# data-mermaid/mermaid-classifier

Measured on AMD Instinct MI355X. Metric: patches/sec (224x224 EfficientNet-B0), higher is better.
Workload: dtype f16; 1 GPU; EfficientNet-B0 forward, batch=256 random 224x224 u8 patches per GPU -> (256,1280) fp32; per_gpu_batch=256, global_batch=256, weights=synthetic seed 0, input_batches_rotated=8, lanes_per_gpu=2, parallelism=patch-sharded x1

## Files before the change

### mermaid_classifier_amd/csrc/device_common.h

```cpp
#pragma once
#include <hip/hip_runtime.h>
#include <stdint.h>
#include <stdlib.h>
#include <algorithm>
#include <atomic>
#include <type_traits>

#include "kernels.h"

typedef _Float16 h8 __attribute__((ext_vector_type(8)));
typedef _Float16 h4 __attribute__((ext_vector_type(4)));
typedef float f4 __attribute__((ext_vector_type(4)));
typedef float f2 __attribute__((ext_vector_type(2)));

static __device__ __forceinline__ float sigmoid_f(float x) { return __builtin_amdgcn_rcpf(1.0f + __expf(-x)); }
static __device__ __forceinline__ float silu_f(float x) { return x * sigmoid_f(x); }
static __device__ __forceinline__ float silu_scaled(float t)
{
    return t * __builtin_amdgcn_rcpf(1.0f + __builtin_amdgcn_exp2f(-t));
}

static __device__ __forceinline__ uint32_t cvt_pk_f16(float a, float b)
{
    uint32_t d;
// ... 87 lines not shown
typedef uint32_t u4v __attribute__((ext_vector_type(4)));
template <typename T>
static __device__ __forceinline__ const GLOBAL_AS T* sgpr_ptr(const void* p)
{
    const uint64_t v = reinterpret_cast<uint64_t>(p);
    const uint32_t lo = __builtin_amdgcn_readfirstlane((uint32_t)v), hi = __builtin_amdgcn_readfirstlane((uint32_t)(v >> 32));
    return reinterpret_cast<const GLOBAL_AS T*>(((uint64_t)hi << 32) | lo);
}
template <typename T>
static __device__ __forceinline__ T gload(const GLOBAL_AS void* base, unsigned byte_off)
{
    return *reinterpret_cast<const GLOBAL_AS T*>(reinterpret_cast<const GLOBAL_AS char*>(base) + byte_off);
}
#define T7_BAR() asm volatile("s_waitcnt lgkmcnt(0)\n\ts_barrier" ::: "memory")

#define LAUNCH_CHECK()                          \
    do {                                        \
        hipError_t e__ = hipGetLastError();     \
        if (e__ != hipSuccess) return (int)e__; \
    } while (0)

template <auto Kernel>
static int set_max_lds(int bytes)
{
    static std::atomic<bool> done[64];
    int dev = 0;
    if (hipGetDevice(&dev) != hipSuccess) dev = 0;
    const bool tracked = dev >= 0 && dev < 64;
    if (tracked && done[dev].load(std::memory_order_acquire)) return 0;
    const hipError_t e = hipFuncSetAttribute(reinterpret_cast<const void*>(Kernel), hipFuncAttributeMaxDynamicSharedMemorySize, bytes);
// ... 32 lines not shown
```

### mermaid_classifier_amd/csrc/k_early.hip

```cpp
#include "device_common.h"

template <int KSTEPS, bool RES>
__global__ __launch_bounds__(256) void thin_proj_kernel(const _Float16* __restrict__ X, int K, const _Float16* __restrict__ Wp,
                                                        const float* __restrict__ bias, _Float16* __restrict__ Y, int N,
                                                        const float* __restrict__ gate, int HW, int frags_per_wg,
                                                        const _Float16* __restrict__ res, int plane_rows)
{
    const int tid = threadIdx.x, lane = tid & 63, wave = tid >> 6;
    const int m = lane & 15, q = lane >> 4;
    const int b = blockIdx.y;
    const int nfrag = HW >> 4;
    const int f0 = blockIdx.x * frags_per_wg;
    const int f1 = f0 + frags_per_wg < nfrag ? f0 + frags_per_wg : nfrag;
    const int cbase = q * 8;
    const int cres = cbase < N ? cbase : 0;
    const _Float16* xb = X + (size_t)b * HW * K;
    auto load = [&](int f, h8 (&dst)[KSTEPS], h8& r) {
        const size_t row = (size_t)f * 16 + m;
#pragma unroll
        for (int ks = 0; ks < KSTEPS; ++ks) {
            const int k0 = ks * 32 + q * 8, k = k0 < K ? k0 : K - 8;
            dst[ks] = plane_rows ? *reinterpret_cast<const h8*>(X + (((size_t)(k >> 5) * plane_rows + (size_t)b * HW + row) * 32 + (k & 31)))
                                 : *reinterpret_cast<const h8*>(xb + row * K + k);
        }
        if (RES) r = *reinterpret_cast<const h8*>(res + ((size_t)b * HW + row) * N + cres);
    };
    h8 xc[KSTEPS], xn[KSTEPS], rc = {0, 0, 0, 0, 0, 0, 0, 0}, rn = rc;
    int f = f0 + wave;
    load(f < f1 ? f : f1 - 1, xc, rc);
    h8 wf[KSTEPS][2];
    {
        f4 g0[KSTEPS], g1[KSTEPS];
        uint4 wr[KSTEPS][2];
#pragma unroll
        for (int ks = 0; ks < KSTEPS; ++ks) {
            const int k0 = ks * 32 + q * 8, k = k0 < K ? k0 : K - 8;
            g0[ks] = *reinterpret_cast<const f4*>(gate + (size_t)b * K + k);
            g1[ks] = *reinterpret_cast<const f4*>(gate + (size_t)b * K + k + 4);
        }
#pragma unroll
        for (int ks = 0; ks < KSTEPS; ++ks)
#pragma unroll
            for (int t = 0; t < 2; ++t) wr[ks][t] = *reinterpret_cast<const uint4*>(Wp + ((size_t)(ks * 2 + t) * 64 + lane) * 8);
#pragma unroll
        for (int ks = 0; ks < KSTEPS; ++ks)
#pragma unroll
// ... 17 lines not shown
#pragma unroll
            for (int j = 0; j < 4; ++j) {
                o[j] = (_Float16)(a0[j] + (RES ? (float)rc[j] : 0.f));
                o[4 + j] = (_Float16)(a1[j] + (RES ? (float)rc[4 + j] : 0.f));
            }
            *reinterpret_cast<h8*>(Y + ((size_t)b * HW + (size_t)f * 16 + m) * N + cbase) = o;
        }
        if (more) {
#pragma unroll
            for (int ks = 0; ks < KSTEPS; ++ks) xc[ks] = xn[ks];
            rc = rn;
        }
    }
}

template <bool PLANAR>
__global__ __launch_bounds__(512, 4) void mb1_kernel(Mb1Args a)
{
    constexpr int WC = 58, NPOS = 17 * WC, NPF = (NPOS + 15) / 16, ES2 = 160;
    extern __shared__ __attribute__((aligned(16))) unsigned char smem[];
    unsigned char* E = smem;
    float* pred = reinterpret_cast<float*>(smem + NPF * 8 * ES2);
    const int tid = threadIdx.x, lane = tid & 63, wave = __builtin_amdgcn_readfirstlane(tid >> 6);
    const int m = lane & 15, q = lane >> 4;
    const int tile = blockIdx.x, b = blockIdx.z;
    const int ty = tile >> 1, tx = tile & 1;
    const int oy0 = 8 * ty, ox0 = 28 * tx, iy0 = 16 * ty, ix0 = 56 * tx;
    const GLOBAL_AS _Float16* xg = sgpr_ptr<_Float16>(a.X) + (size_t)b * 112 * 112 * 32;
    uint2 xbp[8];
    {
        u4v xr[8];
#pragma unroll
        for (int i = 0; i < 8; ++i) {
            const int pf = wave + 8 * i;
            const int p = 16 * pf + m;
            const int r = p / WC, c = p - r * WC;
            const int iy = iy0 + r, ix = ix0 + c;
            const bool ok = pf < NPF && p < NPOS && iy < 112 && ix < 112;
            xr[i] = gload<u4v>(xg, (unsigned)((((ok ? iy : 0) * 112 + (ok ? ix : 0)) * 32 + 8 * q) * 2));
        }
        const uint4 wraw = *reinterpret_cast<const uint4*>(a.pre_w + lane * 8);
        const f4 bpre = *reinterpret_cast<const f4*>(a.pre_b + 4 * q);
        const f4 g0 = *reinterpret_cast<const f4*>(a.pre_gate + (size_t)b * 32 + 8 * q);
        const f4 g1 = *reinterpret_cast<const f4*>(a.pre_gate + (size_t)b * 32 + 8 * q + 4);
        const uint4 wgated = gate_h8(wraw, g0, g1);
        const h8 wpre = *reinterpret_cast<const h8*>(&wgated);
#pragma unroll
        for (int i = 0; i < 8; ++i) {
            const f4 x1 = __builtin_amdgcn_mfma_f32_16x16x32_f16(wpre, *reinterpret_cast<const h8*>(&xr[i]), bpre, 0, 0, 0);
            h4 xh;
#pragma unroll
            for (int j = 0; j < 4; ++j) xh[j] = (_Float16)x1[j];
            xbp[i] = *reinterpret_cast<const uint2*>(&xh);
        }
    }
    h4 wexp[2];
    float bexp[2];
    float kdw[9], dbias;
    auto request_chunk = [&](int chunk) {
// ... 828 lines not shown
    __syncthreads();
    if (tid < 32) {
        float sum = 0.f;
#pragma unroll
        for (int s0 = 0; s0 < 64; s0 += 16) {
            float pv[16];
#pragma unroll
            for (int ss = 0; ss < 16; ++ss) pv[ss] = red[(s0 + ss) * 32 + tid];
#pragma unroll
            for (int ss = 0; ss < 16; ++ss) sum += pv[ss];
        }
        pool_part[((size_t)b * 49 + ty * 7 + tx) * 32 + tid] = sum;
    }
}

template <int KSTEPS, bool RES>
static int launch_thin_proj_t(const GemmArgs& a, hipStream_t st)
{
    const int nfrag = a.HW / 16, patches = a.M / a.HW;
    int per = (int)(((long)nfrag * patches / 2048 + 3) / 4 * 4);
    if (per < 8) per = 8;
    if (per > 112) per = 112;
    if (nfrag < per) per = nfrag;
    dim3 grid((nfrag + per - 1) / per, patches);
    hipLaunchKernelGGL((thin_proj_kernel<KSTEPS, RES>), grid, dim3(256), 0, st, a.X, a.K, a.Wp, a.bias, a.Y, a.N, a.gate, a.HW, per, a.res,
                       a.x_plane_rows);
    LAUNCH_CHECK();
    return 0;
}

#define TP(KSTEPS, RES) {{KSTEPS, RES}, "thin_proj", launch_thin_proj_t<KSTEPS, RES != 0>},
static const Inst<2, GemmArgs> THIN_PROJ_TABLE[] = {TP(1, 1) TP(2, 0) TP(3, 0) TP(5, 0) TP(5, 1)};
#undef TP

const char* thin_proj_label(int ksteps, int res) { return inst_label(THIN_PROJ_TABLE, {ksteps, res}); }

int launch_thin_proj(const GemmArgs& a, int patches, hipStream_t st)
{
    if (a.nt != 2 || a.n_chunks != 1 || a.K > 192 || (a.K & 7) || a.N > 32 || (a.N & 7) || (a.HW & 15) || !a.gate || a.epi != EPI_LINEAR ||
        a.M != patches * a.HW || (a.x_plane_rows && (a.x_plane_rows != a.M || (a.K & 31))))
        return -15;
    return inst_launch(THIN_PROJ_TABLE, {a.Kp / 32, a.res ? 1 : 0}, a, st, -15);
}

int launch_stem_dw(const uint8_t* patches, const _Float16* w, const float* bias, const float* padval, const float* Wdw,
                   const float* bdw, _Float16* out, float* pool_part, int B, hipStream_t st)
{
    hipLaunchKernelGGL(stem_dw_kernel, dim3(7, 7, B), dim3(256), 0, st, patches, w, bias, padval, Wdw, bdw, out, pool_part);
    LAUNCH_CHECK();
    return 0;
}

int launch_mb1(const Mb1Args& a, hipStream_t st)
{
    if (a.B < 1) return -15;
    const int lds = 62 * 8 * 160 + 16 * 32 * 4;
    if (int r = set_max_lds<&mb1_kernel<false>>(lds)) return r;
    if (int r = set_max_lds<&mb1_kernel<true>>(lds)) return r;
    if (a.planar) hipLaunchKernelGGL(mb1_kernel<true>, dim3(14, 1, a.B), dim3(512), lds, st, a);
    else hipLaunchKernelGGL(mb1_kernel<false>, dim3(14, 1, a.B), dim3(512), lds, st, a);
    LAUNCH_CHECK();
    return 0;
}

template <int KSD, int CKS, int CE, int HIMG>
static int launch_mbt_t(const MbtArgs& a, hipStream_t st)
{
    constexpr int NROWS = 14 + 2 * (KSD / 2), WW = HIMG == 28 ? 28 : 30, NPF = (NROWS * WW + 15) / 16;
    const int lds = NPF * 16 * 112 + 10 * 48 * 4;
    if (int r = set_max_lds<&mbt_kernel<KSD, CKS, CE, HIMG>>(lds)) return r;
    hipLaunchKernelGGL((mbt_kernel<KSD, CKS, CE, HIMG>), dim3((HIMG / 14) * (HIMG / 28), CE / 48, a.B), dim3(512), lds, st, a);
    LAUNCH_CHECK();
    return 0;
}

template <int CKS, int CE>
static int launch_mbt4_t(const MbtArgs& a, hipStream_t st)
// ... 46 lines not shown
```

### mermaid_classifier_amd/csrc/k_generic.hip

```cpp
#include "device_common.h"

#define STEM_TILE 16
#define STEM_IN (2 * STEM_TILE + 1)
#define STEM_ROWH 104

template <int NT>
__global__ __launch_bounds__(256) void stem_conv_kernel(const uint8_t* __restrict__ patches,
                                                        const _Float16* __restrict__ w,
                                                        const float* __restrict__ bias,
                                                        const float* __restrict__ padval,
                                                        _Float16* __restrict__ out)
{
    __shared__ __attribute__((aligned(16))) _Float16 tile[STEM_IN * STEM_ROWH];
    const int tx = blockIdx.x, ty = blockIdx.y, b = blockIdx.z;
    const int tid = threadIdx.x;
    const uint8_t* img = patches + (size_t)b * (224 * 224 * 3);
    const int iy0 = ty * 32, ix0 = tx * 32;
    const float pv0 = padval[0], pv1 = padval[1], pv2 = padval[2];
    for (int i = tid; i < STEM_IN * 25; i += 256) {
        const int r = i / 25, d = i - r * 25;
        const int iy = iy0 + r;
        const int boff = ix0 * 3 + d * 4;
        uint32_t word = 0;
        const bool row_ok = iy < 224;
// ... 561 lines not shown
                *reinterpret_cast<f4*>(gate + (size_t)row * C + n) = o;
            }
        }
    }
}

__global__ __launch_bounds__(256) void se_small_kernel(const float* __restrict__ pool_part, int nparts, int C, int Cs,
                                                       const float* __restrict__ wr,
                                                       const float* __restrict__ br,
                                                       const float* __restrict__ we,
                                                       const float* __restrict__ be,
                                                       float* __restrict__ gate)
{
    __shared__ float pooled[256];
    __shared__ float rs[16];
    const int tid = threadIdx.x, lane = tid & 63, wave = tid >> 6;
    const int b = blockIdx.x;
    if (tid < C) {
        const float* pp = pool_part + (size_t)b * nparts * C + tid;
        float s0 = 0.f, s1 = 0.f, s2 = 0.f, s3 = 0.f;
        int p = 0;
#pragma unroll 4
        for (; p + 3 < nparts; p += 4) {
            s0 += pp[(size_t)p * C];
            s1 += pp[(size_t)(p + 1) * C];
            s2 += pp[(size_t)(p + 2) * C];
            s3 += pp[(size_t)(p + 3) * C];
        }
        for (; p < nparts; ++p) s0 += pp[(size_t)p * C];
        pooled[tid] = (s0 + s1) + (s2 + s3);
    }
    __syncthreads();
    for (int j = wave; j < Cs; j += 4) {
        float s = 0.f;
        for (int c = lane; c < C; c += 64) s = __builtin_fmaf(pooled[c], wr[(size_t)j * C + c], s);
#pragma unroll
        for (int o = 32; o >= 1; o >>= 1) s += __shfl_xor(s, o);
        if (lane == 0) rs[j] = silu_f(s + br[j]);
    }
    __syncthreads();
    if (tid < C) {
        float acc = be[tid];
        for (int j = 0; j < Cs; ++j) acc = __builtin_fmaf(rs[j], we[(size_t)tid * Cs + j], acc);
        gate[(size_t)b * C + tid] = sigmoid_f(acc);
    }
}

__global__ __launch_bounds__(1024) void se_wide_kernel(const float* __restrict__ pool_part, int nparts, int C, int Cs,
                                                      const float* __restrict__ wr,
                                                      const float* __restrict__ br,
                                                      const float* __restrict__ we,
                                                      const float* __restrict__ be,
                                                      float* __restrict__ gate)
{
    extern __shared__ float se_sm[];
    float* pooled = se_sm;
    float* rs = se_sm + C;
    const int tid = threadIdx.x, lane = tid & 63, wave = tid >> 6;
    const int b = blockIdx.x;
    for (int c = tid; c < C; c += 1024) {
// ... 573 lines not shown
```

### mermaid_classifier_amd/csrc/kernels.h

```cpp
#pragma once
#include <hip/hip_runtime.h>
#include <stdint.h>

enum { EPI_SILU = 0, EPI_LINEAR = 1, EPI_GAP = 2 };


int mmc_fail(int code, const char* fmt, ...);

struct GemmArgs {
    const _Float16* X;
    int M, K;
    const _Float16* Wp;
    int Kp;
    const float* bias;
    _Float16* Y;
    int N;
    int mt, nt, n_chunks, defer_gate;
    int epi;
    const float* gate;
    int HW;
    const _Float16* res;
    float* gap_out;
    int x_plane_rows;
    float inv_hw;
};

struct Fp8GemmArgs {
    const _Float16* X;
    int M, K;
    const uint8_t* W8;
    int KS128, NFp;
    const float* sw;
    const float* bias;
    _Float16* Y;
    int N;
    const float* gate;
    int HW;
    const _Float16* res;
// ... 64 lines not shown
    const _Float16* pre_wproj;
    const float* pre_bproj;
    const _Float16* head_w;
    const float* head_b;
    float* feat;
    float inv_hw;
    int in_wide;
};
int launch_tail7(const TailArgs& a, hipStream_t st);

struct Mb1Args {
    const _Float16* X;
    const _Float16* pre_w;
    const float* pre_b;
    const float* pre_gate;
    const _Float16* wexp;
    const float* bexp;
    const float* wdw;
    const float* bdw;
    _Float16* D;
    int planar;
    float* pool;
    int B;
};
int launch_mb1(const Mb1Args& a, hipStream_t st);

struct MbtArgs {
    const _Float16* X;
    const _Float16* wexp;
    const float* bexp;
// ... 46 lines not shown
const char* proj_patch_label(int K, int N, int HW, int res);

int launch_mbconv_a(const MbArgs& a, hipStream_t st);
const char* mbconv_a_label(const MbArgs& a);
const char* mbconv_pre_label(const MbArgs& a);
const char* mbconv_d_label(const MbArgs& a);
int launch_mbconv_pre(const MbArgs& a, const _Float16* pre_w, const float* pre_b, const float* pre_gate, hipStream_t st);
int launch_mbconv_d(const MbArgs& a, hipStream_t st);
int launch_stem(const uint8_t* patches, const _Float16* w, const float* bias, const float* padval, _Float16* out, int B,
                int channels, hipStream_t st);
int launch_stem_dw(const uint8_t* patches, const _Float16* w, const float* bias, const float* padval, const float* Wdw,
                   const float* bdw, _Float16* out, float* pool_part, int B, hipStream_t st);
int launch_pw_gemm(const GemmArgs& a, hipStream_t st);
const char* pw_gemm_label(int mt, int nt, int epi, int gate, int res, int defer_gate);
int launch_thin_proj(const GemmArgs& a, int patches, hipStream_t st);
const char* thin_proj_label(int ksteps, int res);
int launch_dwconv(const DwArgs& a, hipStream_t st);
const char* dwconv_label(int ks, int stride, int tw);
int launch_se_gate(const float* pool_part, int nparts, int B, int C, int Cs4, const float* WrP, const float* br,
                   const float* WeP, const float* be, float* gate, hipStream_t st);
int launch_se_small(const float* pool_part, int nparts, int B, int C, int Cs, const float* wr, const float* br,
                    const float* we, const float* be, float* gate, hipStream_t st);
int launch_se_wide(const float* pool_part, int nparts, int B, int C, int Cs, const float* wr, const float* br,
                   const float* we_t , const float* be, float* gate, hipStream_t st);
int launch_mlp_layer(const float* X, int M, int K, const float* W, const float* bias, float* Y, int N, bool relu,
                     hipStream_t st);
int launch_calibrate(const float* logits, int M, int K, const float* a, const float* b, float* proba, int32_t* argmax,
                     hipStream_t st);
int launch_calibrate_topk(const float* logits, int M, int K, const float* a, const float* b, int k, int32_t* idx, float* scores,
                          float* proba, float* rowbuf, hipStream_t st);
constexpr int EVAL_TOTALS = 5;
// ... 5 lines not shown
```

### mermaid_classifier_amd/csrc/mmc_api.cpp

```cpp
#include <hip/hip_runtime.h>

#include <algorithm>
#include <cmath>
#include <cstdarg>
#include <cstdio>
#include <cstdlib>
#include <cstring>
#include <map>
#include <mutex>
#include <thread>
#include <string>
#include <vector>

#include "../../include/mmc.h"
#include "kernels.h"
#include "trainer_internal.h"

static thread_local char g_err[512] = "";
static int fail(int code, const char* fmt, ...)
{
    va_list ap;
    va_start(ap, fmt);
    vsnprintf(g_err, sizeof g_err, fmt, ap);
    va_end(ap);
// ... 123 lines not shown
    if (small_m) {
        int best = 4, waste = 1 << 30;
        for (int nt = 4; nt >= 2; --nt) {
            const int w = (tiles + nt - 1) / nt * nt - tiles;
            if (w < waste) { waste = w; best = nt; }
        }
        return tiles <= 4 ? tiles : best;
    }
    for (int nt = 8; nt >= 1; --nt)
        if (tiles % nt == 0) return nt;
    return 1;
}

struct Options {
    bool keep, graph, tail_clk, profile_serial;
    bool fuse, fuse_b0, mb1, mbt, mbt2, mbt4, mb_dot2, mid14, mid14m, projse, se_small, thin_proj, b1_planar;
    bool tail, tail_full, tail_b11;
    int lanes, fp8_maxh;
};
static bool env_starts(const char* name, char c)
{
    const char* e = getenv(name);
    return e && e[0] == c;
}
static Options read_options()
{
    auto on = [](const char* name) { return !env_starts(name, '0'); };
    Options o;
    o.keep = env_starts("MMC_KEEP_ACTIVATIONS", '1');
    o.graph = on("MMC_GRAPH") && !o.keep;
    o.tail_clk = env_starts("MMC_TAIL_CLK", '1') && !o.keep;
    o.profile_serial = env_starts("MMC_PROFILE_SERIAL", '1');
    o.fuse = on("MMC_FUSE");
    o.fuse_b0 = on("MMC_FUSE_B0");
    o.mb1 = on("MMC_MB1");
    o.mbt = on("MMC_MBT");
    o.mbt2 = on("MMC_MBT2");
    o.mbt4 = on("MMC_MBT4");
    o.mb_dot2 = on("MMC_MB_DOT2");
    o.projse = on("MMC_PROJSE");
    o.se_small = on("MMC_SE_SMALL");
    o.thin_proj = on("MMC_THIN_PROJ");
    o.b1_planar = on("MMC_B1_PLANAR");
    o.tail = on("MMC_TAIL");
    o.tail_full = on("MMC_TAIL_FULL");
    o.tail_b11 = on("MMC_TAIL_B11");
    const char* e = getenv("MMC_MID14");
    o.mid14 = !e || atoi(e) != 0;
    e = getenv("MMC_MID14M");
    o.mid14m = !e || atoi(e) >= 1;
    e = getenv("MMC_LANES");
    o.lanes = e ? atoi(e) : 2;
    e = getenv("MMC_FP8_MAXH");
    o.fp8_maxh = e && atoi(e) > 7 ? atoi(e) : 7;
    return o;
}
// ... 24 lines not shown
    B11All,
};

struct BlockW {
    BlockDef d;
    int H = 0, Ho = 0, ce = 0, cs = 0, cs4 = 0, pad = 0;
    bool has_expand = false, skip = false;
    int tw = 0, CG = 0, S = 0, iters = 0, parts = 0, nz = 1;
    bool fusable = false;
    bool d_fits = false;
    int d_npair = 0, d_wl_off = 0, d_red_off = 0, d_lds = 0;
    MbArgs mb{};
    Front front = Front::Unfused;
    Back back = Back::SeProject;
    Se se = Se::Fused;
    Proj proj = Proj::Gemm;
    bool mbt4 = false, mid14m = false;
    bool planar = false;
    int nparts = 0;
    const char *front_label = nullptr, *back_label = nullptr;
    PwLayer expand, project;
    Fp8Layer p8;
    float *dw_w = nullptr, *dw_b = nullptr;
    float *se_br = nullptr, *se_be = nullptr;
    float *se_wrp = nullptr, *se_wep = nullptr;
    float *se_wr_nat = nullptr, *se_we_nat = nullptr, *se_br_nat = nullptr;
    _Float16* exp_nat = nullptr;
    _Float16* exp_frag = nullptr;
    uint32_t* t_dwp = nullptr;
    uint32_t* t_dwp4 = nullptr;
// ... 92 lines not shown
};

#define MMC_GRAPH_CACHE 32

struct mmc_backbone {
    int device = 0, max_batch = 0;
    int arch = MMC_ARCH_B0, nblk = 16, stem_ch = 32, head_in = 320, feat = 1280;
    Options opt;
    _Float16* stem_w = nullptr;
    float *stem_b = nullptr, *stem_pad = nullptr;
    std::vector<BlockW> blk;
    PwLayer head;
    struct Lane {
        _Float16 *act0 = nullptr, *act1 = nullptr, *expbuf = nullptr, *dwbuf = nullptr;
        float *pool_part = nullptr, *gate = nullptr;
        hipStream_t stream = nullptr;
        hipEvent_t done = nullptr;
    };
    Lane lanes[4];
    struct GraphEntry { const void* in; float* out; int n; hipGraphExec_t exec; };
    std::vector<GraphEntry> graphs;
    bool use_graph = false;
    int graph_warm = 0;
    struct SeenKey { const void* in; float* out; int n; };
    std::vector<SeenKey> seen;
    std::vector<SeenKey> evicted;
    int evictions = 0;
    long long captures = 0;
    hipStream_t gstream = nullptr;
    int nlanes = 1, lane_cap = 0;
// ... 201 lines not shown
        break;
    }
    if (family && !B.front_label)
        return fail(MMC_ERR_ARG, "block %d: no %s instantiation for %dx%d, kernel %d, stride %d, %d -> %d channels (tile %dx%d, chunk %d)",
                    i, family, B.H, B.H, B.d.k, B.d.s, B.d.cin, B.ce, B.mb.TH, B.mb.TWo, B.mb.CC);
    const bool fp8_blk = bb->fp8 && B.Ho <= o.fp8_maxh;
    const char* pp = proj_patch_label(B.ce, B.d.cout, HWo, B.skip ? 1 : 0);
    const bool proj_patch = o.fuse && o.projse && B.fusable && B.has_expand && B.cs4 <= 28 && pp && (is_b0 ? i >= 3 && i <= 10 : !fp8_blk);
    if (tail_blk || (i == 11 && bb->tail == TailRoute::B11)) B.back = Back::Tail;
    else if (proj_patch) B.back = Back::ProjPatch;
    else if (i == 0 && bb->fuse_b0b1) B.back = Back::SeFolded;
    else B.back = Back::SeProject;
    B.back_label = B.back == Back::ProjPatch ? pp : nullptr;
    B.se = !is_b0 ? Se::Wide : (o.se_small && B.ce <= 256 && B.cs <= 16) ? Se::Small : Se::Fused;
    PwLayer& P = B.project;
    const bool thin = o.thin_proj && P.nt == 2 && P.n_chunks == 1 && thin_proj_label(P.Kp / 32, B.skip ? 1 : 0) && P.N <= 32 &&
                      (P.N & 7) == 0 && (HWo & 15) == 0 && HWo >= 3136;
    B.proj = thin ? Proj::Thin : fp8_blk ? Proj::Fp8 : Proj::Gemm;
    if (B.back == Back::SeProject && B.proj == Proj::Gemm && !plan_gemm(P, EPI_LINEAR, true, B.skip, HWo))
        return fail(MMC_ERR_ARG, "block %d: no pw_gemm (project) instantiation for %d -> %d channels at %dx%d", i, B.ce, B.d.cout, B.Ho, B.Ho);
    B.planar = B.front == Front::Mb1 && thin && o.b1_planar && !o.keep && P.K == 96;
    return 0;
}

extern "C" int mmc_backbone_create_ex(const void* packed, size_t nbytes, int arch, int device, int max_batch, unsigned flags,
                                      mmc_backbone** out)
{
    if (!out) return fail(MMC_ERR_ARG, "out is NULL");
    if (flags & ~(unsigned)MMC_PRECISION_FP8) return fail(MMC_ERR_ARG, "unknown flags 0x%x", flags);
    if ((flags & MMC_PRECISION_FP8) && arch != MMC_ARCH_B4)
        return fail(MMC_ERR_ARG, "MMC_PRECISION_FP8 is implemented for MMC_ARCH_B4 (BASELINE configs[4]): B0's late blocks run fused kernels without a separate project GEMM");
    *out = nullptr;
    if (!packed || nbytes < 16) return fail(MMC_ERR_WEIGHTS, "weights blob is empty");
    if (arch != MMC_ARCH_B0 && arch != MMC_ARCH_B4) return fail(MMC_ERR_ARG, "unsupported arch %d (MMC_ARCH_B0 or MMC_ARCH_B4)", arch);
    if (max_batch < 1 || max_batch > 4096) return fail(MMC_ERR_ARG, "max_batch %d out of range [1,4096]", max_batch);
    const uint8_t* base = static_cast<const uint8_t*>(packed);
    uint32_t hdr[4];
// ... 51 lines not shown
        const std::vector<BlockW>& K = bb->blk;
        bb->fuse_stem = is_b0 && o.fuse;
        const MbArgs& m1 = K[1].mb;
        bb->fuse_b0b1 = o.fuse_b0 && bb->fuse_stem && K[0].ce == 32 && K[0].d.cout == 16 && K[1].d.cin == 16 && K[1].fusable &&
                        !(o.mb_dot2 && B0_DOT2[1] && K[1].d_fits) && m1.TH == 8 && m1.TWo == 8 && m1.CC == 48 && m1.tw == 2 &&
                        m1.pb == 1 && m1.npair == 3;
        bool t12 = is_b0 && o.fuse && o.tail && NBLK == 16;
        for (int i = 12; i <= 15 && t12; ++i)
            t12 = K[i].fusable && K[i].H == 7 && K[i].d.s == 1 && K[i].d.cin == 192 && K[i].ce == 1152 && K[i].cs == 48;
        const BlockW& B11 = K[11 < NBLK ? 11 : 0];
        const bool t11 = t12 && o.tail_full && HEAD_IN % 32 == 0 && B11.fusable && B11.ce == 672 && B11.d.cout == 192 &&
                         B11.cs4 == 28 && B11.mb.tiles_x * B11.mb.tiles_y == 1;
        const bool t11all = t11 && o.tail_b11 && !o.keep && B11.mb.ksteps == 4 && B11.d.k == 5 && B11.d.s == 2 && B11.H == 14;
        bb->tail = t11all ? TailRoute::B11All : t11 ? TailRoute::B11 : t12 ? TailRoute::B12 : TailRoute::None;
        for (int i = 0; i < NBLK; ++i) TRY_OR_FREE(plan_block(bb, bb->blk[i], i));
        bb->head.nt = 4;
        const int HWh = K[NBLK - 1].Ho * K[NBLK - 1].Ho;
        if (bb->tail != TailRoute::B11 && bb->tail != TailRoute::B11All && !plan_gemm(bb->head, EPI_GAP, false, false, HWh)) {
            mmc_backbone_destroy(bb);
            return fail(MMC_ERR_ARG, "head: no pw_gemm (average pool) instantiation for nt %d at %d pixels per patch", bb->head.nt, HWh);
        }
    }

    std::vector<uint64_t> table(2 * (size_t)nt);
    memcpy(table.data(), base + 16, (size_t)nt * 16);
    BlobReader rd{base, nbytes, nt, table.data()};
    int err = 0;
#define TAKE(var, n, what)                         \
    const float* var = rd.take((n), what, &err);   \
    if (!var) { mmc_backbone_destroy(bb); return err; }
// ... 260 lines not shown
    }
    const size_t mb = (size_t)max_batch;
    {
        int nl = std::max(1, std::min(o.lanes, 4));
        if (bb->keep || max_batch < 2 * nl) nl = 1;
        bb->nlanes = nl;
        bb->lane_cap = (max_batch + nl - 1) / nl;
        const size_t lc = (size_t)bb->lane_cap;
        for (int l = 0; l < nl; ++l) {
            mmc_backbone::Lane& L = bb->lanes[l];
            TRY_OR_FREE(dev_alloc(bb, &L.act0, lc * max_act));
            TRY_OR_FREE(dev_alloc(bb, &L.act1, lc * max_act));
            TRY_OR_FREE(dev_alloc(bb, &L.expbuf, lc * (max_exp ? max_exp : 64)));
            TRY_OR_FREE(dev_alloc(bb, &L.dwbuf, lc * max_dw));
            TRY_OR_FREE(dev_alloc(bb, &L.pool_part, lc * max_pool));
            TRY_OR_FREE(dev_alloc(bb, &L.gate, lc * (size_t)max_c));
            if (nl > 1) {
                if (hipStreamCreateWithFlags(&L.stream, hipStreamNonBlocking) != hipSuccess ||
                    hipEventCreateWithFlags(&L.done, hipEventDisableTiming) != hipSuccess) {
                    mmc_backbone_destroy(bb);
                    return fail(MMC_ERR_HIP, "cannot create internal stream/event");
                }
            }
        }
        if (nl > 1 && hipEventCreateWithFlags(&bb->fork, hipEventDisableTiming) != hipSuccess) {
            mmc_backbone_destroy(bb);
            return fail(MMC_ERR_HIP, "cannot create fork event");
        }
    }
    TRY_OR_FREE(dev_alloc(bb, &bb->in_stage, mb * (size_t)IMG * IMG * 3));
// ... 69 lines not shown
    _Float16* y = ws.act1;
    auto swap_xy = [&] { _Float16* t = x; x = y; y = t; };
    const int lane_idx = (int)(&ws - bb->lanes);
    if (!bb->fuse_stem) {
        STEP("stem", "stem_conv", launch_stem(patches_dev, bb->stem_w, bb->stem_b, bb->stem_pad, x, n, bb->stem_ch, st));
        SAVE("stem", x, (size_t)n * 112 * 112 * bb->stem_ch, true);
    }
    for (int i = 0; i < bb->nblk; ++i) {
        BlockW& B = bb->blk[i];
        if (B.front == Front::Tail) break;
        const int HWi = B.H * B.H, HWo = B.Ho * B.Ho;
        snprintf(nm, sizeof nm, "b%d.mbconv", i);
        switch (B.front) {
        case Front::StemDw:
            STEP("stem+b0.dw", "stem_dw", launch_stem_dw(patches_dev, bb->stem_w, bb->stem_b, bb->stem_pad, B.dw_w, B.dw_b,
                                                          bb->fuse_b0b1 ? y : ws.dwbuf, ws.pool_part, n, st));
            break;
        case Front::Mbt: {
            MbtArgs ta{};
            ta.X = x; ta.wexp = B.exp_frag; ta.bexp = B.expand.b; ta.dwp = B.t_dwp; ta.bdw = B.dw_b; ta.D = ws.dwbuf;
            ta.pool = ws.pool_part; ta.B = n; ta.H = B.H; ta.Cin = B.d.cin; ta.Ce = B.ce; ta.ks = B.d.k; ta.stride = B.d.s;
            ta.dwtoe = B.mbt4 ? B.dw_diag : nullptr;
            STEP(nm, B.front_label, launch_mbt(ta, st));
            break;
        }
        case Front::Mid14: {
            Mid14Args ma{};
            ma.X = x; ma.wexp = B.exp_frag; ma.bexp = B.expand.b; ma.dwp = B.t_dwp4; ma.bdw = B.dw_b; ma.D = ws.dwbuf;
            ma.pool = ws.pool_part; ma.B = n; ma.Cin = B.d.cin; ma.Ce = B.ce; ma.ks = B.d.k;
            ma.dwdiag = B.mid14m ? B.dw_diag : nullptr;
            ma.nsplit = B.mid14m ? 1 : 4;
            if (bb->mid_clk && i == 10) ma.dbg_clk = bb->mid_clk + (size_t)lane_idx * bb->lane_cap * 128;
            STEP(nm, B.front_label, launch_mid14(ma, st));
            break;
        }
        case Front::Mb1: {
            Mb1Args m1{};
            m1.X = y; m1.pre_w = bb->b0_pre_w; m1.pre_b = bb->blk[0].project.b; m1.pre_gate = ws.gate; m1.wexp = bb->b1_exp_pre;
            m1.bexp = B.expand.b; m1.wdw = B.dw_w; m1.bdw = B.dw_b; m1.D = ws.dwbuf; m1.pool = ws.pool_part; m1.B = n;
            m1.planar = B.planar ? 1 : 0;
            STEP("b0.project+b1.mbconv", "mb1", launch_mb1(m1, st));
            break;
        }
        case Front::MbPre: case Front::MbD: case Front::MbA: {
            MbArgs a = B.mb;
            a.X = x; a.Wexp = B.exp_nat; a.bexp = B.expand.b; a.Wdw = B.dw_w; a.bdw = B.dw_b; a.out = ws.dwbuf;
            a.pool_part = ws.pool_part; a.B = n;
            if (B.front == Front::MbD) {
                STEP(nm, B.front_label, launch_mbconv_d(a, st));
            } else if (B.front == Front::MbPre) {
                a.X = y; a.Cin = 32; a.Wexp = bb->b1_exp_pre;
                STEP("b0.project+b1.mbconv", B.front_label, launch_mbconv_pre(a, bb->b0_pre_w, bb->blk[0].project.b, ws.gate, st));
            } else {
                STEP(nm, B.front_label, launch_mbconv_a(a, st));
            }
            break;
// ... 26 lines not shown
            pa.dbg_clk = bb->keep ? bb->dbg_clk : nullptr;
            pa.B = n; pa.HW = HWo; pa.K = B.ce; pa.N = B.d.cout; pa.CSP = B.cs4; pa.nparts = B.nparts;
            pa.psc = (float)(1.0 / ((double)HWo * LOG2E));
            snprintf(nm, sizeof nm, "b%d.projse", i);
            STEP(nm, B.back_label, launch_proj_patch(pa, st));
            snprintf(nm, sizeof nm, "b%d.gate", i);
            SAVE(nm, ws.gate, (size_t)n * B.ce, false);
            snprintf(nm, sizeof nm, "b%d.out", i);
            SAVE(nm, y, (size_t)n * HWo * B.d.cout, true);
            snprintf(nm, sizeof nm, "b%d.clk", i);
            SAVE(nm, bb->dbg_clk, (size_t)n * 8, false);
            swap_xy();
            continue;
        }
        snprintf(nm, sizeof nm, "b%d.gate", i);
        if (B.se == Se::Wide)
            STEP(nm, "se_wide", launch_se_wide(ws.pool_part, B.nparts, n, B.ce, B.cs, B.se_wr_nat, B.se_br_nat, B.se_we_nat, B.se_be,
                                               ws.gate, st));
        else if (B.se == Se::Small)
            STEP(nm, "se_small", launch_se_small(ws.pool_part, B.nparts, n, B.ce, B.cs, B.se_wr_nat, B.se_br_nat, B.se_we_nat, B.se_be,
                                                 ws.gate, st));
        else
            STEP(nm, "se_fused", launch_se_gate(ws.pool_part, B.nparts, n, B.ce, B.cs4, B.se_wrp, B.se_br, B.se_wep, B.se_be,
                                                ws.gate, st));
        SAVE(nm, ws.gate, (size_t)n * B.ce, false);
        if (B.back == Back::SeFolded) continue;
        snprintf(nm, sizeof nm, "b%d.project", i);
        if (B.proj == Proj::Thin) {
            GemmArgs a{};
            a.X = ws.dwbuf; a.M = n * HWo; a.K = B.project.K; a.Wp = B.project.w; a.Kp = B.project.Kp; a.bias = B.project.b; a.Y = y;
            a.N = B.project.N; a.nt = B.project.nt; a.n_chunks = B.project.n_chunks; a.epi = EPI_LINEAR; a.gate = ws.gate; a.HW = HWo;
            a.res = B.skip ? x : nullptr;
            a.x_plane_rows = B.planar ? n * HWo : 0;
            STEP(nm, "thin_proj", launch_thin_proj(a, n, st));
        } else if (B.proj == Proj::Fp8) {
            Fp8GemmArgs fa{};
            fa.X = ws.dwbuf; fa.M = n * HWo; fa.K = B.p8.K; fa.W8 = B.p8.w8; fa.KS128 = B.p8.KS128; fa.NFp = B.p8.NFp; fa.sw = B.p8.sw;
            fa.bias = B.p8.b; fa.Y = y; fa.N = B.p8.N; fa.gate = ws.gate; fa.HW = HWo; fa.res = B.skip ? x : nullptr;
            STEP(nm, "pw_gemm_fp8", launch_pw_gemm_fp8(fa, st));
        } else
            STEP(nm, B.project.label[gemm_mt(B.project, n * HWo) - 1],
                 run_gemm(B.project, ws.dwbuf, n * HWo, y, EPI_LINEAR, ws.gate, HWo, B.skip ? x : nullptr, nullptr, st));
        snprintf(nm, sizeof nm, "b%d.out", i);
        SAVE(nm, y, (size_t)n * HWo * B.d.cout, true);
        swap_xy();
    }
    const float inv_hw7 = (float)(1.0 / (49.0 * LOG2E));
    if (bb->tail == TailRoute::B11All || (bb->tail == TailRoute::B11 && !bb->keep)) {
        const BlockW& B11 = bb->blk[11];
// ... 755 lines not shown
```

Baseline: 229,000 patches/s.

## Inline small squeeze-excite gate into thin projection and mb1 kernels

Adds an option that computes the small SE gate (pool reduce, reduce FC, SiLU, expand FC, sigmoid) inside each consuming workgroup of the thin projection kernel (blocks 1 and 2) and the fused b0-project+b1 kernel. This removes the separate se_small launches and the gate round-trip through global memory. In exchange, every workgroup redundantly recomputes the per-patch gate and adds LDS barriers before its main loop. The path is gated behind the MMC_SE_INLINE environment flag, and the standalone se_small kernel is refactored to share the same chain code.

```diff
diff --git a/mermaid_classifier_amd/csrc/device_common.h b/mermaid_classifier_amd/csrc/device_common.h
--- a/mermaid_classifier_amd/csrc/device_common.h
+++ b/mermaid_classifier_amd/csrc/device_common.h
@@ -125,6 +125,108 @@
 }
 #define T7_BAR() asm volatile("s_waitcnt lgkmcnt(0)\n\ts_barrier" ::: "memory")
 
+template <bool SPREAD>
+static __device__ __forceinline__ int se_small_part(int i, int k, int nparts)
+{
+    if (!SPREAD) return i;
+    const int ng = nparts >> 2;
+    return i < ng ? 4 * i + k : 4 * ng + (i - ng);
+}
+
+template <int NT, bool SPREAD, typename FP, typename FWR, typename FBR, typename FWE, typename FBE, typename FOUT>
+static __device__ __forceinline__ void se_small_chain(int tid, int nparts, int C, int Cs, FP part, FWR wr, FBR br, FWE we, FBE be,
+                                                      float* pooled, float* rs, FOUT out)
+{
+    constexpr int NW = NT / 64;
+    const int lane = tid & 63, wave = tid >> 6;
+    const int ng = nparts >> 2, nrem = nparts & 3;
+    if (SPREAD) {
+        const int c = tid >> 2, k = tid & 3;
+        if (c < C) {
+            float s = 0.f;
+#pragma unroll
+            for (int i = 0; i < ng; ++i) s += part(i);
+#pragma unroll
+            for (int r = 0; r < nrem; ++r)
+                if (k == 0) s += part(ng + r);
+            s = quad_sum(s);
+            if (k == 0) pooled[c] = s;
+        }
+    } else if (tid < C) {
+        float s0 = 0.f, s1 = 0.f, s2 = 0.f, s3 = 0.f;
+#pragma unroll 4
+        for (int g = 0; g < ng; ++g) {
+            s0 += part(4 * g);
+            s1 += part(4 * g + 1);
+            s2 += part(4 * g + 2);
+            s3 += part(4 * g + 3);
+        }
+#pragma unroll
+        for (int r = 0; r < nrem; ++r) s0 += part(4 * ng + r);
+        pooled[tid] = (s0 + s1) + (s2 + s3);
+    }
+    T7_BAR();
+#pragma unroll
+    for (int ji = 0; ji * NW < Cs; ++ji) {
+        const int j = wave + ji * NW;
+        if (j < Cs) {
+            float s = 0.f;
+#pragma unroll
+            for (int ci = 0; ci * 64 < C; ++ci) {
+                const int c = lane + 64 * ci;
+                if (c < C) s = __builtin_fmaf(pooled[c], wr(ji, ci, j, c), s);
+            }
+#pragma unroll
+            for (int o = 32; o >= 1; o >>= 1) s += __shfl_xor(s, o);
+            if (lane == 0) rs[j] = silu_f(s + br(ji, j));
+        }
+    }
+    T7_BAR();
+    if (tid < C) {
+        float acc = be();
+#pragma unroll
+        for (int j = 0; j < Cs; ++j) acc = __builtin_fmaf(rs[j], we(j), acc);
+        out(tid, sigmoid_f(acc));
+    }
+}
+
+template <int NT, bool SPREAD, int C, int CS, int NP>
+struct SeSmallRegs {
+    static constexpr int NW = NT / 64, NSEQ = SPREAD ? NP / 4 + NP % 4 : NP, NJ = (CS + NW - 1) / NW, NC = (C + 63) / 64;
+    static_assert(!SPREAD || 4 * C <= NT, "SPREAD: one thread per channel and chain");
+    static_assert(C <= NT && CS <= 16, "se_small_chain's limits");
+    float part[NSEQ], wr[NJ][NC], br[NJ], we[CS], be;
+    __device__ __forceinline__ void request(int tid, const float* __restrict__ pp, const float* __restrict__ wr_g,
+                                            const float* __restrict__ br_g, const float* __restrict__ we_g, const float* __restrict__ be_g)
+    {
+        const int lane = tid & 63, wave = tid >> 6;
+        const int cs = SPREAD ? tid >> 2 : tid, c = cs < C ? cs : C - 1;
+#pragma unroll
+        for (int i = 0; i < NSEQ; ++i) part[i] = pp[se_small_part<SPREAD>(i, tid & 3, NP) * C + c];
+#pragma unroll
+        for (int ji = 0; ji < NJ; ++ji) {
+            const int js = wave + ji * NW, j = js < CS ? js : CS - 1;
+#pragma unroll
+            for (int ci = 0; ci < NC; ++ci) {
+                const int c1 = lane + 64 * ci;
+                wr[ji][ci] = wr_g[j * C + (c1 < C ? c1 : C - 1)];
+            }
+            br[ji] = br_g[j];
+        }
+        const int c2 = tid < C ? tid : C - 1;
+#pragma unroll
+        for (int j = 0; j < CS; ++j) we[j] = we_g[c2 * CS + j];
+        be = be_g[c2];
+    }
+    template <typename FOUT>
+    __device__ __forceinline__ void run(int tid, float* pooled, float* rs, FOUT out)
+    {
+        se_small_chain<NT, SPREAD>(
+            tid, NP, C, CS, [&](int i) { return part[i]; }, [&](int ji, int ci, int, int) { return wr[ji][ci]; },
+            [&](int ji, int) { return br[ji]; }, [&](int j) { return we[j]; }, [&]() { return be; }, pooled, rs, out);
+    }
+};
+
 #define LAUNCH_CHECK()                          \
     do {                                        \
         hipError_t e__ = hipGetLastError();     \
diff --git a/mermaid_classifier_amd/csrc/k_early.hip b/mermaid_classifier_amd/csrc/k_early.hip
--- a/mermaid_classifier_amd/csrc/k_early.hip
+++ b/mermaid_classifier_amd/csrc/k_early.hip
@@ -1,10 +1,15 @@
 #include "device_common.h"
 
-template <int KSTEPS, bool RES>
+struct ThinSeArgs {
+    const float* pool_part;
+    const float *wr, *br, *we, *be;
+    float* dbg_gate;
+};
+template <int KSTEPS, bool RES, bool SE = false>
 __global__ __launch_bounds__(256) void thin_proj_kernel(const _Float16* __restrict__ X, int K, const _Float16* __restrict__ Wp,
                                                         const float* __restrict__ bias, _Float16* __restrict__ Y, int N,
                                                         const float* __restrict__ gate, int HW, int frags_per_wg,
-                                                        const _Float16* __restrict__ res, int plane_rows)
+                                                        const _Float16* __restrict__ res, int plane_rows, ThinSeArgs se_a)
 {
     const int tid = threadIdx.x, lane = tid & 63, wave = tid >> 6;
     const int m = lane & 15, q = lane >> 4;
@@ -29,7 +34,33 @@
     int f = f0 + wave;
     load(f < f1 ? f : f1 - 1, xc, rc);
     h8 wf[KSTEPS][2];
-    {
+    if constexpr (SE) {
+        static_assert(KSTEPS == 3 || KSTEPS == 5, "SE: B0's block 1 (K = 96) or block 2 (K = 144)");
+        constexpr int C = KSTEPS == 3 ? 96 : 144, CS = KSTEPS == 3 ? 4 : 6, NP = KSTEPS == 3 ? 14 : 8;
+        __shared__ float se_pooled[C], se_rs[16], se_gate[C];
+        SeSmallRegs<256, false, C, CS, NP> se;
+        se.request(tid, se_a.pool_part + (size_t)b * NP * C, se_a.wr, se_a.br, se_a.we, se_a.be);
+        PIN_VMEM();
+        uint4 wr[KSTEPS][2];
+#pragma unroll
+        for (int ks = 0; ks < KSTEPS; ++ks)
+#pragma unroll
+            for (int t = 0; t < 2; ++t) wr[ks][t] = *reinterpret_cast<const uint4*>(Wp + ((size_t)(ks * 2 + t) * 64 + lane) * 8);
+        PIN_VMEM();
+        se.run(tid, se_pooled, se_rs, [&](int c, float g) { se_gate[c] = g; });
+        T7_BAR();
+        if (se_a.dbg_gate && blockIdx.x == 0 && tid < C) se_a.dbg_gate[(size_t)b * C + tid] = se_gate[tid];
+#pragma unroll
+        for (int ks = 0; ks < KSTEPS; ++ks) {
+            const int k0 = ks * 32 + q * 8, k = k0 < C ? k0 : C - 8;
+            const f4 g0 = *reinterpret_cast<const f4*>(se_gate + k), g1 = *reinterpret_cast<const f4*>(se_gate + k + 4);
+#pragma unroll
+            for (int t = 0; t < 2; ++t) {
+                const uint4 gw = gate_h8(wr[ks][t], g0, g1);
+                wf[ks][t] = *reinterpret_cast<const h8*>(&gw);
+            }
+        }
+    } else {
         f4 g0[KSTEPS], g1[KSTEPS];
         uint4 wr[KSTEPS][2];
 #pragma unroll
@@ -77,7 +108,7 @@
     }
 }
 
-template <bool PLANAR>
+template <bool PLANAR, bool SE>
 __global__ __launch_bounds__(512, 4) void mb1_kernel(Mb1Args a)
 {
     constexpr int WC = 58, NPOS = 17 * WC, NPF = (NPOS + 15) / 16, ES2 = 160;
@@ -92,6 +123,14 @@
     const GLOBAL_AS _Float16* xg = sgpr_ptr<_Float16>(a.X) + (size_t)b * 112 * 112 * 32;
     uint2 xbp[8];
     {
+        float* se_pooled = pred;
+        float* se_rs = pred + 32;
+        float* se_gate = pred + 48;
+        SeSmallRegs<512, true, 32, 8, 49> se;
+        if (SE) {
+            se.request(tid, a.pre_pool + (size_t)b * 49 * 32, a.se_wr, a.se_br, a.se_we, a.se_be);
+            PIN_VMEM();
+        }
         u4v xr[8];
 #pragma unroll
         for (int i = 0; i < 8; ++i) {
@@ -104,8 +143,18 @@
         }
         const uint4 wraw = *reinterpret_cast<const uint4*>(a.pre_w + lane * 8);
         const f4 bpre = *reinterpret_cast<const f4*>(a.pre_b + 4 * q);
-        const f4 g0 = *reinterpret_cast<const f4*>(a.pre_gate + (size_t)b * 32 + 8 * q);
-        const f4 g1 = *reinterpret_cast<const f4*>(a.pre_gate + (size_t)b * 32 + 8 * q + 4);
+        f4 g0, g1;
+        if (SE) {
+            PIN_VMEM();
+            se.run(tid, se_pooled, se_rs, [&](int c, float g) { se_gate[c] = g; });
+            T7_BAR();
+            g0 = *reinterpret_cast<const f4*>(se_gate + 8 * q);
+            g1 = *reinterpret_cast<const f4*>(se_gate + 8 * q + 4);
+            if (a.dbg_gate && tile == 0 && tid < 32) a.dbg_gate[(size_t)b * 32 + tid] = se_gate[tid];
+        } else {
+            g0 = *reinterpret_cast<const f4*>(a.pre_gate + (size_t)b * 32 + 8 * q);
+            g1 = *reinterpret_cast<const f4*>(a.pre_gate + (size_t)b * 32 + 8 * q + 4);
+        }
         const uint4 wgated = gate_h8(wraw, g0, g1);
         const h8 wpre = *reinterpret_cast<const h8*>(&wgated);
 #pragma unroll
@@ -964,7 +1013,7 @@
     }
 }
 
-template <int KSTEPS, bool RES>
+template <int KSTEPS, bool RES, bool SE>
 static int launch_thin_proj_t(const GemmArgs& a, hipStream_t st)
 {
     const int nfrag = a.HW / 16, patches = a.M / a.HW;
@@ -973,24 +1022,29 @@
     if (per > 112) per = 112;
     if (nfrag < per) per = nfrag;
     dim3 grid((nfrag + per - 1) / per, patches);
-    hipLaunchKernelGGL((thin_proj_kernel<KSTEPS, RES>), grid, dim3(256), 0, st, a.X, a.K, a.Wp, a.bias, a.Y, a.N, a.gate, a.HW, per, a.res,
-                       a.x_plane_rows);
+    const ThinSeArgs se{a.se_pool, a.se_wr, a.se_br, a.se_we, a.se_be, a.dbg_gate};
+    hipLaunchKernelGGL((thin_proj_kernel<KSTEPS, RES, SE>), grid, dim3(256), 0, st, a.X, a.K, a.Wp, a.bias, a.Y, a.N, a.gate, a.HW, per, a.res,
+                       a.x_plane_rows, se);
     LAUNCH_CHECK();
     return 0;
 }
 
-#define TP(KSTEPS, RES) {{KSTEPS, RES}, "thin_proj", launch_thin_proj_t<KSTEPS, RES != 0>},
-static const Inst<2, GemmArgs> THIN_PROJ_TABLE[] = {TP(1, 1) TP(2, 0) TP(3, 0) TP(5, 0) TP(5, 1)};
+#define TP(KSTEPS, RES, SE) {{KSTEPS, RES, SE}, "thin_proj", launch_thin_proj_t<KSTEPS, RES != 0, SE != 0>},
+static const Inst<3, GemmArgs> THIN_PROJ_TABLE[] = {TP(1, 1, 0) TP(2, 0, 0) TP(3, 0, 0) TP(5, 0, 0) TP(5, 1, 0) TP(3, 0, 1) TP(5, 1, 1)};
 #undef TP
 
-const char* thin_proj_label(int ksteps, int res) { return inst_label(THIN_PROJ_TABLE, {ksteps, res}); }
+const char* thin_proj_label(int ksteps, int res, int se) { return inst_label(THIN_PROJ_TABLE, {ksteps, res, se}); }
 
 int launch_thin_proj(const GemmArgs& a, int patches, hipStream_t st)
 {
-    if (a.nt != 2 || a.n_chunks != 1 || a.K > 192 || (a.K & 7) || a.N > 32 || (a.N & 7) || (a.HW & 15) || !a.gate || a.epi != EPI_LINEAR ||
-        a.M != patches * a.HW || (a.x_plane_rows && (a.x_plane_rows != a.M || (a.K & 31))))
+    const bool se = a.se_pool != nullptr;
+    if (a.nt != 2 || a.n_chunks != 1 || a.K > 192 || (a.K & 7) || a.N > 32 || (a.N & 7) || (a.HW & 15) || (a.gate != nullptr) == se ||
+        a.epi != EPI_LINEAR || a.M != patches * a.HW || (a.x_plane_rows && (a.x_plane_rows != a.M || (a.K & 31))))
         return -15;
-    return inst_launch(THIN_PROJ_TABLE, {a.Kp / 32, a.res ? 1 : 0}, a, st, -15);
+    if (se && (!a.se_wr || !a.se_br || !a.se_we || !a.se_be ||
+               !((a.K == 96 && a.se_cs == 4 && a.se_nparts == 14) || (a.K == 144 && a.se_cs == 6 && a.se_nparts == 8))))
+        return -15;
+    return inst_launch(THIN_PROJ_TABLE, {a.Kp / 32, a.res ? 1 : 0, se ? 1 : 0}, a, st, -15);
 }
 
 int launch_stem_dw(const uint8_t* patches, const _Float16* w, const float* bias, const float* padval, const float* Wdw,
@@ -1004,13 +1058,19 @@
 int launch_mb1(const Mb1Args& a, hipStream_t st)
 {
     if (a.B < 1) return -15;
+    const bool se = a.pre_pool != nullptr;
+    if (se ? (a.pre_gate || a.nparts != 49 || !a.se_wr || !a.se_br || !a.se_we || !a.se_be || a.pre_pool == a.pool) : !a.pre_gate) return -15;
     const int lds = 62 * 8 * 160 + 16 * 32 * 4;
-    if (int r = set_max_lds<&mb1_kernel<false>>(lds)) return r;
-    if (int r = set_max_lds<&mb1_kernel<true>>(lds)) return r;
-    if (a.planar) hipLaunchKernelGGL(mb1_kernel<true>, dim3(14, 1, a.B), dim3(512), lds, st, a);
-    else hipLaunchKernelGGL(mb1_kernel<false>, dim3(14, 1, a.B), dim3(512), lds, st, a);
-    LAUNCH_CHECK();
-    return 0;
+    auto go = [&](auto planar_tag, auto se_tag) {
+        constexpr auto kernel = &mb1_kernel<decltype(planar_tag)::value, decltype(se_tag)::value>;
+        if (int r = set_max_lds<kernel>(lds)) return r;
+        hipLaunchKernelGGL(kernel, dim3(14, 1, a.B), dim3(512), lds, st, a);
+        LAUNCH_CHECK();
+        return 0;
+    };
+    using T = std::true_type;
+    using F = std::false_type;
+    return a.planar ? (se ? go(T{}, T{}) : go(T{}, F{})) : (se ? go(F{}, T{}) : go(F{}, F{}));
 }
 
 template <int KSD, int CKS, int CE, int HIMG>
diff --git a/mermaid_classifier_amd/csrc/k_generic.hip b/mermaid_classifier_amd/csrc/k_generic.hip
--- a/mermaid_classifier_amd/csrc/k_generic.hip
+++ b/mermaid_classifier_amd/csrc/k_generic.hip
@@ -599,36 +599,14 @@
 {
     __shared__ float pooled[256];
     __shared__ float rs[16];
-    const int tid = threadIdx.x, lane = tid & 63, wave = tid >> 6;
+    const int tid = threadIdx.x;
     const int b = blockIdx.x;
-    if (tid < C) {
-        const float* pp = pool_part + (size_t)b * nparts * C + tid;
-        float s0 = 0.f, s1 = 0.f, s2 = 0.f, s3 = 0.f;
-        int p = 0;
-#pragma unroll 4
-        for (; p + 3 < nparts; p += 4) {
-            s0 += pp[(size_t)p * C];
-            s1 += pp[(size_t)(p + 1) * C];
-            s2 += pp[(size_t)(p + 2) * C];
-            s3 += pp[(size_t)(p + 3) * C];
-        }
-        for (; p < nparts; ++p) s0 += pp[(size_t)p * C];
-        pooled[tid] = (s0 + s1) + (s2 + s3);
-    }
-    __syncthreads();
-    for (int j = wave; j < Cs; j += 4) {
-        float s = 0.f;
-        for (int c = lane; c < C; c += 64) s = __builtin_fmaf(pooled[c], wr[(size_t)j * C + c], s);
-#pragma unroll
-        for (int o = 32; o >= 1; o >>= 1) s += __shfl_xor(s, o);
-        if (lane == 0) rs[j] = silu_f(s + br[j]);
-    }
-    __syncthreads();
-    if (tid < C) {
-        float acc = be[tid];
-        for (int j = 0; j < Cs; ++j) acc = __builtin_fmaf(rs[j], we[(size_t)tid * Cs + j], acc);
-        gate[(size_t)b * C + tid] = sigmoid_f(acc);
-    }
+    const int cc = tid < C ? tid : 0;
+    const float* pp = pool_part + (size_t)b * nparts * C + cc;
+    se_small_chain<256, false>(
+        tid, nparts, C, Cs, [&](int p) { return pp[(size_t)p * C]; }, [&](int, int, int j, int c) { return wr[(size_t)j * C + c]; },
+        [&](int, int j) { return br[j]; }, [&](int j) { return we[(size_t)cc * Cs + j]; }, [&]() { return be[cc]; }, pooled, rs,
+        [&](int c, float g) { gate[(size_t)b * C + c] = g; });
 }
 
 __global__ __launch_bounds__(1024) void se_wide_kernel(const float* __restrict__ pool_part, int nparts, int C, int Cs,
diff --git a/mermaid_classifier_amd/csrc/kernels.h b/mermaid_classifier_amd/csrc/kernels.h
--- a/mermaid_classifier_amd/csrc/kernels.h
+++ b/mermaid_classifier_amd/csrc/kernels.h
@@ -22,6 +22,10 @@
     const _Float16* res;
     float* gap_out;
     int x_plane_rows;
+    const float* se_pool;
+    int se_nparts, se_cs;
+    const float *se_wr, *se_br, *se_we, *se_be;
+    float* dbg_gate;
     float inv_hw;
 };
 
@@ -116,6 +120,10 @@
     const _Float16* pre_w;
     const float* pre_b;
     const float* pre_gate;
+    const float* pre_pool;
+    int nparts;
+    const float *se_wr, *se_br, *se_we, *se_be;
+    float* dbg_gate;
     const _Float16* wexp;
     const float* bexp;
     const float* wdw;
@@ -192,7 +200,7 @@
 int launch_pw_gemm(const GemmArgs& a, hipStream_t st);
 const char* pw_gemm_label(int mt, int nt, int epi, int gate, int res, int defer_gate);
 int launch_thin_proj(const GemmArgs& a, int patches, hipStream_t st);
-const char* thin_proj_label(int ksteps, int res);
+const char* thin_proj_label(int ksteps, int res, int se);
 int launch_dwconv(const DwArgs& a, hipStream_t st);
 const char* dwconv_label(int ks, int stride, int tw);
 int launch_se_gate(const float* pool_part, int nparts, int B, int C, int Cs4, const float* WrP, const float* br,
diff --git a/mermaid_classifier_amd/csrc/mmc_api.cpp b/mermaid_classifier_amd/csrc/mmc_api.cpp
--- a/mermaid_classifier_amd/csrc/mmc_api.cpp
+++ b/mermaid_classifier_amd/csrc/mmc_api.cpp
@@ -161,7 +161,7 @@
 
 struct Options {
     bool keep, graph, tail_clk, profile_serial;
-    bool fuse, fuse_b0, mb1, mbt, mbt2, mbt4, mb_dot2, mid14, mid14m, projse, se_small, thin_proj, b1_planar;
+    bool fuse, fuse_b0, mb1, mbt, mbt2, mbt4, mb_dot2, mid14, mid14m, projse, se_small, se_inline, thin_proj, b1_planar;
     bool tail, tail_full, tail_b11;
     int lanes, fp8_maxh;
 };
@@ -187,6 +187,7 @@
     o.mb_dot2 = on("MMC_MB_DOT2");
     o.projse = on("MMC_PROJSE");
     o.se_small = on("MMC_SE_SMALL");
+    o.se_inline = on("MMC_SE_INLINE");
     o.thin_proj = on("MMC_THIN_PROJ");
     o.b1_planar = on("MMC_B1_PLANAR");
     o.tail = on("MMC_TAIL");
@@ -241,6 +242,7 @@
     Front front = Front::Unfused;
     Back back = Back::SeProject;
     Se se = Se::Fused;
+    bool se_inline = false;
     Proj proj = Proj::Gemm;
     bool mbt4 = false, mid14m = false;
     bool planar = false;
@@ -363,6 +365,7 @@
     struct Lane {
         _Float16 *act0 = nullptr, *act1 = nullptr, *expbuf = nullptr, *dwbuf = nullptr;
         float *pool_part = nullptr, *gate = nullptr;
+        float* pool_b0 = nullptr;
         hipStream_t stream = nullptr;
         hipEvent_t done = nullptr;
     };
@@ -594,13 +597,28 @@
     B.back_label = B.back == Back::ProjPatch ? pp : nullptr;
     B.se = !is_b0 ? Se::Wide : (o.se_small && B.ce <= 256 && B.cs <= 16) ? Se::Small : Se::Fused;
     PwLayer& P = B.project;
-    const bool thin = o.thin_proj && P.nt == 2 && P.n_chunks == 1 && thin_proj_label(P.Kp / 32, B.skip ? 1 : 0) && P.N <= 32 &&
+    const bool thin = o.thin_proj && P.nt == 2 && P.n_chunks == 1 && thin_proj_label(P.Kp / 32, B.skip ? 1 : 0, 0) && P.N <= 32 &&
                       (P.N & 7) == 0 && (HWo & 15) == 0 && HWo >= 3136;
     B.proj = thin ? Proj::Thin : fp8_blk ? Proj::Fp8 : Proj::Gemm;
     if (B.back == Back::SeProject && B.proj == Proj::Gemm && !plan_gemm(P, EPI_LINEAR, true, B.skip, HWo))
         return fail(MMC_ERR_ARG, "block %d: no pw_gemm (project) instantiation for %d -> %d channels at %dx%d", i, B.ce, B.d.cout, B.Ho, B.Ho);
     B.planar = B.front == Front::Mb1 && thin && o.b1_planar && !o.keep && P.K == 96;
     return 0;
+}
+
+static void plan_se_inline(mmc_backbone* bb)
+{
+    const Options& o = bb->opt;
+    if (!o.se_inline || bb->arch != MMC_ARCH_B0) return;
+    for (size_t i = 0; i < bb->blk.size(); ++i) {
+        BlockW& B = bb->blk[i];
+        if (B.se != Se::Small) continue;
+        if (i == 0)
+            B.se_inline = B.back == Back::SeFolded && B.front == Front::StemDw && bb->blk[1].front == Front::Mb1 && B.ce == 32 && B.cs == 8;
+        else
+            B.se_inline = B.back == Back::SeProject && B.proj == Proj::Thin && thin_proj_label(B.project.Kp / 32, B.skip ? 1 : 0, 1) &&
+                          ((B.ce == 96 && B.cs == 4 && B.nparts == 14) || (B.ce == 144 && B.cs == 6 && B.nparts == 8));
+    }
 }
 
 extern "C" int mmc_backbone_create_ex(const void* packed, size_t nbytes, int arch, int device, int max_batch, unsigned flags,
@@ -682,6 +700,7 @@
         const bool t11all = t11 && o.tail_b11 && !o.keep && B11.mb.ksteps == 4 && B11.d.k == 5 && B11.d.s == 2 && B11.H == 14;
         bb->tail = t11all ? TailRoute::B11All : t11 ? TailRoute::B11 : t12 ? TailRoute::B12 : TailRoute::None;
         for (int i = 0; i < NBLK; ++i) TRY_OR_FREE(plan_block(bb, bb->blk[i], i));
+        plan_se_inline(bb);
         bb->head.nt = 4;
         const int HWh = K[NBLK - 1].Ho * K[NBLK - 1].Ho;
         if (bb->tail != TailRoute::B11 && bb->tail != TailRoute::B11All && !plan_gemm(bb->head, EPI_GAP, false, false, HWh)) {
@@ -972,6 +991,7 @@
             TRY_OR_FREE(dev_alloc(bb, &L.expbuf, lc * (max_exp ? max_exp : 64)));
             TRY_OR_FREE(dev_alloc(bb, &L.dwbuf, lc * max_dw));
             TRY_OR_FREE(dev_alloc(bb, &L.pool_part, lc * max_pool));
+            if (bb->blk[0].se_inline) TRY_OR_FREE(dev_alloc(bb, &L.pool_b0, lc * 49 * 32));
             TRY_OR_FREE(dev_alloc(bb, &L.gate, lc * (size_t)max_c));
             if (nl > 1) {
                 if (hipStreamCreateWithFlags(&L.stream, hipStreamNonBlocking) != hipSuccess ||
@@ -1071,7 +1091,7 @@
         switch (B.front) {
         case Front::StemDw:
             STEP("stem+b0.dw", "stem_dw", launch_stem_dw(patches_dev, bb->stem_w, bb->stem_b, bb->stem_pad, B.dw_w, B.dw_b,
-                                                          bb->fuse_b0b1 ? y : ws.dwbuf, ws.pool_part, n, st));
+                                                          bb->fuse_b0b1 ? y : ws.dwbuf, B.se_inline ? ws.pool_b0 : ws.pool_part, n, st));
             break;
         case Front::Mbt: {
             MbtArgs ta{};
@@ -1096,7 +1116,13 @@
             m1.X = y; m1.pre_w = bb->b0_pre_w; m1.pre_b = bb->blk[0].project.b; m1.pre_gate = ws.gate; m1.wexp = bb->b1_exp_pre;
             m1.bexp = B.expand.b; m1.wdw = B.dw_w; m1.bdw = B.dw_b; m1.D = ws.dwbuf; m1.pool = ws.pool_part; m1.B = n;
             m1.planar = B.planar ? 1 : 0;
+            const BlockW& B0 = bb->blk[0];
+            if (B0.se_inline) {
+                m1.pre_gate = nullptr; m1.pre_pool = ws.pool_b0; m1.nparts = B0.nparts; m1.se_wr = B0.se_wr_nat; m1.se_br = B0.se_br_nat;
+                m1.se_we = B0.se_we_nat; m1.se_be = B0.se_be; m1.dbg_gate = bb->keep ? ws.gate : nullptr;
+            }
             STEP("b0.project+b1.mbconv", "mb1", launch_mb1(m1, st));
+            if (B0.se_inline) SAVE("b0.gate", ws.gate, (size_t)n * B0.ce, false);
             break;
         }
         case Front::MbPre: case Front::MbD: case Front::MbA: {
@@ -1153,7 +1179,9 @@
             continue;
         }
         snprintf(nm, sizeof nm, "b%d.gate", i);
-        if (B.se == Se::Wide)
+        if (B.se_inline)
+            ;
+        else if (B.se == Se::Wide)
             STEP(nm, "se_wide", launch_se_wide(ws.pool_part, B.nparts, n, B.ce, B.cs, B.se_wr_nat, B.se_br_nat, B.se_we_nat, B.se_be,
                                                ws.gate, st));
         else if (B.se == Se::Small)
@@ -1162,7 +1190,7 @@
         else
             STEP(nm, "se_fused", launch_se_gate(ws.pool_part, B.nparts, n, B.ce, B.cs4, B.se_wrp, B.se_br, B.se_wep, B.se_be,
                                                 ws.gate, st));
-        SAVE(nm, ws.gate, (size_t)n * B.ce, false);
+        if (!B.se_inline) SAVE(nm, ws.gate, (size_t)n * B.ce, false);
         if (B.back == Back::SeFolded) continue;
         snprintf(nm, sizeof nm, "b%d.project", i);
         if (B.proj == Proj::Thin) {
@@ -1171,7 +1199,15 @@
             a.N = B.project.N; a.nt = B.project.nt; a.n_chunks = B.project.n_chunks; a.epi = EPI_LINEAR; a.gate = ws.gate; a.HW = HWo;
             a.res = B.skip ? x : nullptr;
             a.x_plane_rows = B.planar ? n * HWo : 0;
+            if (B.se_inline) {
+                a.gate = nullptr; a.se_pool = ws.pool_part; a.se_nparts = B.nparts; a.se_cs = B.cs; a.se_wr = B.se_wr_nat; a.se_br = B.se_br_nat;
+                a.se_we = B.se_we_nat; a.se_be = B.se_be; a.dbg_gate = bb->keep ? ws.gate : nullptr;
+            }
             STEP(nm, "thin_proj", launch_thin_proj(a, n, st));
+            if (B.se_inline) {
+                snprintf(nm, sizeof nm, "b%d.gate", i);
+                SAVE(nm, ws.gate, (size_t)n * B.ce, false);
+            }
         } else if (B.proj == Proj::Fp8) {
             Fp8GemmArgs fa{};
             fa.X = ws.dwbuf; fa.M = n * HWo; fa.K = B.p8.K; fa.W8 = B.p8.w8; fa.KS128 = B.p8.KS128; fa.NFp = B.p8.NFp; fa.sw = B.p8.sw;
```

Result: slower. 225,300 patches/s (-1.6%).
